# gnosisguild/pvw-rs

Measured on AMD Instinct MI355X. Metric: parties/s for n-party encrypt (pvw::crypto::encrypt); achieved HBM GB/s vs peak, higher is better.
Workload: dtype u64

## Files before the change

### include/pvw_hip.h

```cpp
#ifndef PVW_HIP_H
#define PVW_HIP_H

#include <stddef.h>
#include <stdint.h>

#if defined(__GNUC__)
#define PVW_API __attribute__((visibility("default")))
#else
#define PVW_API
#endif

#ifdef __cplusplus
extern "C" {
#endif

typedef struct pvw_ctx pvw_ctx;

enum {
  PVW_OK = 0,
  PVW_ERR_INVALID_PARAMETERS = 1,
  PVW_ERR_SAMPLING = 2,
  PVW_ERR_ENCRYPTION = 3,
  PVW_ERR_DECRYPTION = 4,
  PVW_ERR_KEY_GENERATION = 5,
// ... 209 lines not shown
PVW_API int32_t pvw_ntt_inverse(pvw_ctx* ctx, uint64_t* polys, size_t count);
PVW_API int32_t pvw_small_to_poly(pvw_ctx* ctx, const int64_t* coeffs, size_t count, uint64_t* polys,
                          uint32_t repr);

PVW_API int32_t pvw_sample_cbd(pvw_ctx* ctx, const uint8_t seed[32], uint32_t domain, uint32_t index0,
                       size_t count, float variance, int64_t* out);
PVW_API int32_t pvw_sample_uniform(pvw_ctx* ctx, const uint8_t seed[32], uint32_t domain,
                           uint32_t index0, size_t count, uint64_t bound, int64_t* out);
PVW_API int32_t pvw_sample_gaussian(pvw_ctx* ctx, const uint8_t seed[32], uint32_t index0, size_t count,
                            uint64_t bound, int64_t* out );

PVW_API int32_t pvw_ctx_set_profiling(pvw_ctx* ctx, int32_t on);
PVW_API int32_t pvw_ctx_kernel_time(pvw_ctx* ctx, const char* name, double* total_ms, uint64_t* launches);
PVW_API int32_t pvw_ctx_reset_profiling(pvw_ctx* ctx);
PVW_API int32_t pvw_host_alloc(size_t bytes, void** out);
PVW_API int32_t pvw_host_free(void* p);

PVW_API int32_t pvw_ctx_resident_bytes(const pvw_ctx* ctx, uint64_t* crs_bytes, uint64_t* pk_bytes);
PVW_API int32_t pvw_ctx_derived_bytes(const pvw_ctx* ctx, uint64_t* packed_bytes, uint64_t* mfma_tiled_bytes);

enum { PVW_PREPARE_PACKED = 1, PVW_PREPARE_MFMA = 2, PVW_PREPARE_SUM = 4 };
PVW_API int32_t pvw_prepare(pvw_ctx* ctx, uint32_t flags, void* stream, uint64_t* bytes_out);
PVW_API int32_t pvw_ctx_packed_active(const pvw_ctx* ctx, uint32_t* width_out);
PVW_API int32_t pvw_ctx_synchronize(pvw_ctx* ctx);

PVW_API int32_t pvw_wire_poly_bytes(const pvw_ctx* ctx, size_t* out);
PVW_API int32_t pvw_wire_header(const pvw_ctx* ctx, uint32_t kind, uint32_t repr, uint32_t lo, uint32_t hi, uint32_t lo2,
                                uint32_t hi2, uint8_t* out, size_t cap, size_t* len);
PVW_API int32_t pvw_wire_header_check(const pvw_ctx* ctx, const uint8_t* data, size_t len, uint32_t* kind, uint32_t* repr,
                                      uint32_t* ranges, size_t* header_len);
PVW_API int32_t pvw_wire_pack(pvw_ctx* ctx, const uint64_t* polys, size_t count, uint8_t* out);
PVW_API int32_t pvw_wire_pack_device(pvw_ctx* ctx, const uint64_t* d_polys, size_t count, uint8_t* d_out, void* stream);
PVW_API int32_t pvw_wire_unpack(pvw_ctx* ctx, const uint8_t* data, size_t count, uint64_t* polys);
PVW_API int32_t pvw_wire_unpack_device(pvw_ctx* ctx, const uint8_t* d_in, size_t count, uint64_t* d_polys, uint64_t* d_bad,
                                       void* stream);
PVW_API int32_t pvw_wire_pack_host(const pvw_ctx* ctx, const uint64_t* polys, size_t count, uint8_t* out);
PVW_API int32_t pvw_wire_unpack_host(const pvw_ctx* ctx, const uint8_t* data, size_t count, uint64_t* polys, uint64_t* bad_out);
PVW_API int32_t pvw_load_pk_wire(pvw_ctx* ctx, uint32_t party_lo, uint32_t party_hi, const uint8_t* body, uint32_t repr);
PVW_API int32_t pvw_get_pk_wire(pvw_ctx* ctx, uint32_t party_lo, uint32_t party_hi, uint8_t* body_out, uint32_t repr);
PVW_API int32_t pvw_load_crs_wire(pvw_ctx* ctx, const uint8_t* body, uint32_t repr);
PVW_API int32_t pvw_get_crs_wire(pvw_ctx* ctx, uint8_t* body_out, uint32_t repr);

#ifdef __cplusplus
}
#endif
#endif
// ... 1 lines not shown
```

### pvw_rs_amd/_ffi.py

```python
from __future__ import annotations

import ctypes as C
import os

HERE = os.path.dirname(os.path.abspath(__file__))
LIB_PATH = os.path.join(HERE, "libpvw_hip.so")

PVW_OK = 0
ERROR_NAMES = {
    1: "InvalidParameters", 2: "SamplingError", 3: "EncryptionError", 4: "DecryptionError",
    5: "KeyGenerationError", 6: "CrsError", 7: "SerializationError", 8: "DeserializationError",
    9: "EncodingError", 10: "DecodingError", 11: "ValidationError", 12: "ContextError",
    13: "PolynomialError", 14: "MatrixError", 15: "DimensionMismatch", 16: "IndexOutOfBounds",
    17: "InsufficientData", 18: "InvalidFormat", 19: "InternalError",
}
REPR_POWER, REPR_NTT = 0, 1
RND_SEED, RND_EXPLICIT = 0, 1
DOM_R, DOM_E1, DOM_E2, DOM_SK, DOM_EKEY, DOM_CRS, DOM_GAUSS, DOM_PK, DOM_CALL = range(9)
PREPARE_PACKED, PREPARE_MFMA, PREPARE_SUM = 1, 2, 4
WIRE_PARAMS, WIRE_CRS, WIRE_PK, WIRE_CT, WIRE_SK = 1, 2, 3, 4, 5


class pvw_params_t(C.Structure):
    _fields_ = [
# ... 86 lines not shown
    "pvw_selftest_decode_fixed": [_P, _P, C.c_size_t, _P],
    "pvw_selftest_mfma_i8": [_P, _P, _P, _P],
    "pvw_selftest_secret_residue": [_P, C.POINTER(C.c_uint64), C.POINTER(C.c_uint64)],
    "pvw_selftest_siphash": [_P, C.c_size_t, C.c_uint64, C.c_uint64, C.c_int32, C.c_int32, C.POINTER(C.c_uint64)],
    "pvw_selftest_decode_tables": [_P, C.POINTER(C.c_uint32)],
    "pvw_selftest_decode_shortcuts": [_P, _P, C.c_size_t, _P, _P],
    "pvw_build_is_tuning": [],
    "pvw_crs_seed_from_tag": [C.c_char_p, _P],
    "pvw_ntt_forward": [_P, _P, C.c_size_t],
    "pvw_ntt_inverse": [_P, _P, C.c_size_t],
    "pvw_small_to_poly": [_P, _P, C.c_size_t, _P, C.c_uint32],
    "pvw_sample_cbd": [_P, _P, C.c_uint32, C.c_uint32, C.c_size_t, C.c_float, _P],
    "pvw_sample_uniform": [_P, _P, C.c_uint32, C.c_uint32, C.c_size_t, C.c_uint64, _P],
    "pvw_sample_gaussian": [_P, _P, C.c_uint32, C.c_size_t, C.c_uint64, _P],
    "pvw_ctx_set_profiling": [_P, C.c_int32],
    "pvw_ctx_kernel_time": [_P, C.c_char_p, C.POINTER(C.c_double), C.POINTER(C.c_uint64)],
    "pvw_ctx_reset_profiling": [_P],
    "pvw_host_alloc": [C.c_size_t, C.POINTER(_P)],
    "pvw_host_free": [_P],
    "pvw_ctx_resident_bytes": [_P, C.POINTER(C.c_uint64), C.POINTER(C.c_uint64)],
    "pvw_ctx_derived_bytes": [_P, C.POINTER(C.c_uint64), C.POINTER(C.c_uint64)],
    "pvw_prepare": [_P, C.c_uint32, _P, C.POINTER(C.c_uint64)],
    "pvw_ctx_packed_active": [_P, C.POINTER(C.c_uint32)],
    "pvw_ctx_synchronize": [_P],
    "pvw_wire_poly_bytes": [_P, C.POINTER(C.c_size_t)],
    "pvw_wire_header": [_P, C.c_uint32, C.c_uint32, C.c_uint32, C.c_uint32, C.c_uint32, C.c_uint32, _P, C.c_size_t,
                        C.POINTER(C.c_size_t)],
    "pvw_wire_header_check": [_P, _P, C.c_size_t, C.POINTER(C.c_uint32), C.POINTER(C.c_uint32), _P, C.POINTER(C.c_size_t)],
    "pvw_wire_pack": [_P, _P, C.c_size_t, _P],
    "pvw_wire_pack_device": [_P, _P, C.c_size_t, _P, _P],
    "pvw_wire_unpack": [_P, _P, C.c_size_t, _P],
    "pvw_wire_unpack_device": [_P, _P, C.c_size_t, _P, _P, _P],
    "pvw_wire_pack_host": [_P, _P, C.c_size_t, _P],
    "pvw_wire_unpack_host": [_P, _P, C.c_size_t, _P, C.POINTER(C.c_uint64)],
    "pvw_load_pk_wire": [_P, C.c_uint32, C.c_uint32, _P, C.c_uint32],
    "pvw_get_pk_wire": [_P, C.c_uint32, C.c_uint32, _P, C.c_uint32],
    "pvw_load_crs_wire": [_P, _P, C.c_uint32],
    "pvw_get_crs_wire": [_P, _P, C.c_uint32],
}

_TUNING_SIGNATURES = {
    "pvw_selftest_read_bandwidth": [_P, C.c_uint32, _P, _P],
    "pvw_tuning_read_stamps": [_P, _P, _P, C.c_uint32],
    "pvw_tuning_read_probe": [_P, C.c_uint32, C.c_uint32, C.c_uint32, C.c_uint32, _P, _P],
}

# ... 45 lines not shown
```

### pvw_rs_amd/api.py

```python
from __future__ import annotations

import ctypes as C
import struct
from typing import List, Optional, Sequence, Tuple

import numpy as np

from . import _ffi
from ._ffi import REPR_NTT, REPR_POWER


class PvwError(Exception):

    def __init__(self, code: int, message: str):
        self.code = code
        self.variant = _ffi.ERROR_NAMES.get(code, f"Unknown({code})")
        super().__init__(f"{self.variant}: {message}")


def _check(rc: int, lib=None) -> None:
    if rc != _ffi.PVW_OK:
        raise PvwError(rc, _ffi.last_error(lib))


# ... 239 lines not shown

    def reset_profiling(self) -> None:
        self._call("pvw_ctx_reset_profiling")

    def kernel_time(self, name: str) -> Tuple[float, int]:
        ms, cnt = C.c_double(), C.c_uint64()
        self._call("pvw_ctx_kernel_time", name.encode(), C.byref(ms), C.byref(cnt))
        return ms.value, cnt.value

    def resident_bytes(self) -> Tuple[int, int]:
        a, b = C.c_uint64(), C.c_uint64()
        self._call("pvw_ctx_resident_bytes", C.byref(a), C.byref(b))
        return a.value, b.value

    def prepare(self, flags: int = _ffi.PREPARE_PACKED | _ffi.PREPARE_MFMA, stream=None) -> int:
        taken = C.c_uint64(0)
        self._call("pvw_prepare", int(flags), C.c_void_p(stream) if stream else None, C.byref(taken))
        return int(taken.value)

    def packed_active(self) -> int:
        w = C.c_uint32(0)
        self._call("pvw_ctx_packed_active", C.byref(w))
        return int(w.value)

    def derived_bytes(self) -> Tuple[int, int]:
        a, b = C.c_uint64(0), C.c_uint64(0)
        self._call("pvw_ctx_derived_bytes", C.byref(a), C.byref(b))
        return int(a.value), int(b.value)

    def synchronize(self) -> None:
        self._call("pvw_ctx_synchronize")

    def wire_poly_bytes(self) -> int:
        out = C.c_size_t()
        self._call("pvw_wire_poly_bytes", C.byref(out))
        return int(out.value)

    def to_bytes(self) -> bytes:
        return bytes(_wire_header(self, _ffi.WIRE_PARAMS))

    @staticmethod
    def from_bytes(data, device: int = -1) -> "PvwParameters":
        raw = bytes(data[:_WIRE_FIXED]) if len(data) >= _WIRE_FIXED else b""
        if len(raw) < _WIRE_FIXED or raw[:4] != _WIRE_MAGIC:
            raise PvwError(18, "wire: truncated header or bad magic")
        version, kind = struct.unpack_from("<HH", raw, 4)
# ... 898 lines not shown
```

### pvw_rs_amd/csrc/pvw_capi.hip

```cpp
#include <hip/hip_runtime.h>

#include <atomic>
#include <cmath>
#include <cstdio>
#include <cstring>
#include <functional>
#include <map>
#include <mutex>
#include <string>
#include <thread>
#include <vector>

#include "../../include/pvw_hip.h"
#include "pvw_arith.h"
#include "pvw_bignum.h"
#include "pvw_chacha.h"
#include "pvw_decode.h"
#include "pvw_kernels.h"
#if PVW_TUNING
#include "../../include/pvw_hip_tuning.h"
#endif

using namespace pvw;

// ... 135 lines not shown
  std::vector<u64> tw, itw, linv, ghat, gpow;
  bool roots_locked = false;
  std::vector<u64> dec_words;
  DecodeTables dec_host{};
  DecodeTables dec_dev{};
  void* d_dec = nullptr;

  std::atomic<bool> dev_ready{false};
  void* d_tables = nullptr;
  DevTables dt{};
  u64* dA = nullptr;
  u64* dB = nullptr;
  u64* xmA = nullptr;
  u64* xmB = nullptr;
  bool xm_valid = false;
  u64* pkA = nullptr;
  u64* pkB = nullptr;
  u32* pk_flag = nullptr;
  u32 pk_width = 0;
  bool pkA_valid = false, pkB_valid = false;
  bool pk_wide = false;
  u32 pk_nomem_calls = 0;
  bool crs_loaded = false;
  u32 num_keys = 0;
  hipStream_t stream = nullptr;

  std::mutex mu, init_mu;
  std::vector<Workspace*> pool;
  std::map<void*, Workspace*> async_ws;

  bool profiling = false;
  std::vector<ProfRec> prof;
  std::map<std::string, std::pair<double, uint64_t>> prof_acc;

  u32 rowsA() const { return c1_hi - c1_lo; }
  u32 rowsB() const { return party_hi - party_lo; }
  u32 R() const { return 128 / l; }
  size_t poly() const { return (size_t)L * l; }
  size_t tiled_words(u32 rows) const { return (size_t)((rows + R() - 1) / R()) * L * k * 128; }
};

struct ProfScope {
  pvw_ctx* c;
  hipStream_t s;
  ProfRec rec;
  bool on;
// ... 460 lines not shown
  pvw_ctx* c = new pvw_ctx();
  c->n = p->n; c->k = p->k; c->l = p->l; c->L = p->num_moduli;
  c->moduli.assign(p->moduli, p->moduli + p->num_moduli);
  c->variance = p->secret_variance;
  c->b1 = p->error_bound_1; c->b2 = p->error_bound_2;
  c->device = p->device;
  c->party_lo = p->party_lo; c->party_hi = p->party_hi;
  c->c1_lo = p->c1_lo; c->c1_hi = p->c1_hi;
  if (c->party_lo == 0 && c->party_hi == 0) c->party_hi = c->n;
  if (c->c1_lo == 0 && c->c1_hi == 0) c->c1_hi = c->k;
  if (c->party_lo > c->party_hi || c->party_hi > c->n || c->c1_lo > c->c1_hi || c->c1_hi > c->k) {
    delete c;
    return fail(PVW_ERR_INVALID_PARAMETERS, "party / c1 shard out of range");
  }
  compute_q_delta(c->moduli.data(), c->L, c->l, c->Q, c->delta, c->delta_pow);
  c->halfQ = c->Q.shr(1);
  for (u32 i = 0; i < c->L; ++i) {
    c->mods.push_back(make_mod(c->moduli[i]));
    c->psi.push_back(min_primitive_root(c->mods[i], 2 * c->l));
    BigInt qi = c->Q / BigInt(c->moduli[i]);
    c->crt_qi.push_back(qi);
    c->crt_inv.push_back(powmod(qi.mod_small(c->moduli[i]), c->moduli[i] - 2, c->mods[i]));
  }
  build_tables(c);
  build_decode_tables(c);
  {
    u32 maxbits = 0;
    for (u64 q : c->moduli) {
      u32 bits = 0;
      for (; q; q >>= 1) ++bits;
      if (bits > maxbits) maxbits = bits;
    }
    c->pk_width = packed_width(maxbits, c->k, c->l);
  }
  *out = c;
  return PVW_OK;
}

int32_t pvw_ctx_destroy(pvw_ctx* c) {
  if (!c) return PVW_OK;
  if (c->dev_ready) {
    hipSetDevice(c->device);
    hipDeviceSynchronize();
    for (auto& r : c->prof) { hipEventDestroy(r.a); hipEventDestroy(r.b); }
    for (Workspace* w : c->pool) ws_free(w);
    for (auto& kv : c->async_ws) ws_free(kv.second);
// ... 285 lines not shown
  PVW_TRY(device_ws(c, stream, &s, &w));
  size_t taken = 0;
  if (flags & PVW_PREPARE_SUM) PVW_TRY(sum_prepare(c, w, s));
  if (flags & PVW_PREPARE_PACKED) (void)ensure_packed(c, s, true, &taken);
  if (flags & PVW_PREPARE_MFMA) {
    const bool had_a = c->xmA != nullptr, had_b = c->xmB != nullptr;
    PVW_TRY(ws_gemm_buffers(c, w));
    PVW_TRY(ensure_xm(c, s));
    if (!had_a && c->xmA) taken += xm_words(c->rowsA(), c->k, c->L, c->l) * 8;
    if (!had_b && c->xmB) taken += xm_words(c->rowsB(), c->k, c->L, c->l) * 8;
  }
  PVW_HIP(hipStreamSynchronize(s));
  if (bytes_out) *bytes_out = taken;
  return PVW_OK;
}

static int32_t check_repr(uint32_t repr) {
  if (repr != PVW_REPR_POWER && repr != PVW_REPR_NTT) return fail(PVW_ERR_INVALID_FORMAT, "unknown representation");
  return PVW_OK;
}

static void matrix_changed(pvw_ctx* c, bool crs) {
  c->xm_valid = false;
  (crs ? c->pkA_valid : c->pkB_valid) = false;
  c->pk_wide = false;
}

int32_t pvw_load_crs(pvw_ctx* c, const uint64_t* a, uint32_t repr) {
  if (!c || !a) return fail(PVW_ERR_INVALID_PARAMETERS, "NULL argument");
  PVW_TRY(check_repr(repr));
  PVW_TRY(ensure_device(c));
  matrix_changed(c, true);
  PVW_TRY(ensure_matrix(c, &c->dA, c->rowsA()));
  PVW_TRY(load_rows_host(c, c->dA, c->c1_lo, c->c1_hi, 0, c->k, a, repr));
  c->crs_loaded = true;
  return PVW_OK;
}
int32_t pvw_load_crs_device(pvw_ctx* c, const uint64_t* d_a, uint32_t repr, void* stream) {
  if (!c || !d_a) return fail(PVW_ERR_INVALID_PARAMETERS, "NULL argument");
  PVW_TRY(check_repr(repr));
  PVW_TRY(ensure_device(c));
  matrix_changed(c, true);
  PVW_TRY(ensure_matrix(c, &c->dA, c->rowsA()));
  PVW_TRY(load_rows_device(c, c->dA, c->c1_lo, c->c1_hi, 0, c->k, d_a, repr, call_stream(c, stream)));
  c->crs_loaded = true;
  return PVW_OK;
}
int32_t pvw_crs_generate(pvw_ctx* c, const uint8_t seed[32]) {
  if (!c || !seed) return fail(PVW_ERR_INVALID_PARAMETERS, "NULL argument");
  PVW_TRY(ensure_device(c));
  matrix_changed(c, true);
  PVW_TRY(ensure_matrix(c, &c->dA, c->rowsA()));
  {
    ProfScope ps(c, "fill_uniform", c->stream);
    PVW_HIP(launch_fill_uniform_tiled(c->dA, make_key(seed), DOM_CRS, c->rowsA(), 0, c->c1_lo, c->k, c->L,
                                      c->l, c->dt, c->stream));
  }
  PVW_HIP(hipStreamSynchronize(c->stream));
  c->crs_loaded = true;
  return PVW_OK;
}
static u64 siphash(const uint8_t* m, size_t len, u64 k0, u64 k1, int c_rounds, int d_rounds) {
  u64 v0 = k0 ^ 0x736f6d6570736575ULL, v1 = k1 ^ 0x646f72616e646f6dULL, v2 = k0 ^ 0x6c7967656e657261ULL,
      v3 = k1 ^ 0x7465646279746573ULL;
  auto rotl = [](u64 x, int b) { return (x << b) | (x >> (64 - b)); };
  auto round = [&]() {
    v0 += v1; v1 = rotl(v1, 13); v1 ^= v0; v0 = rotl(v0, 32);
    v2 += v3; v3 = rotl(v3, 16); v3 ^= v2;
    v0 += v3; v3 = rotl(v3, 21); v3 ^= v0;
    v2 += v1; v1 = rotl(v1, 17); v1 ^= v2; v2 = rotl(v2, 32);
  };
  size_t i = 0;
  for (; i + 8 <= len; i += 8) {
    u64 w = 0;
    for (int b = 0; b < 8; ++b) w |= (u64)m[i + b] << (8 * b);
    v3 ^= w;
    for (int r = 0; r < c_rounds; ++r) round();
    v0 ^= w;
  }
  u64 w = (u64)(len & 0xff) << 56;
  for (int b = 0; i + b < len; ++b) w |= (u64)m[i + b] << (8 * b);
  v3 ^= w;
// ... 408 lines not shown
      pb.job[2].raw_out = w->esmall + (size_t)rA * l;
      es1 = pb.job[1].raw_out;
      es2 = pb.job[2].raw_out;
      pb.njobs = 3;
    }
  } else {
    pb.njobs = 3;
  }
  {
    ProfScope ps(c, "prologue", s);
    PVW_HIP(launch_prologue(pb, c->dt, L, l, s));
  }
  {
    ProfScope ps(c, "mac_rows", s);
    MacSection a(width ? c->pkA : c->dA, compact ? nullptr : d_c1, out_c1, rA), b(width ? c->pkB : c->dB, compact ? nullptr : d_c2, out_c2, rB);
    if (compact) {
      a.e_small = es1;
      b.e_small = es2;
      b.scalars = d_scalars + c->party_lo;
    }
    if (rs) {
      a.rnd_ctr = &rs->counter;
      a.rnd_adv = 1;
    }
    if (width) PVW_HIP(launch_mac_rows_packed(a, b, w->rhat, c->dt, k, L, l, width, s));
    else PVW_HIP(launch_mac_rows(a, b, w->rhat, c->dt, k, L, l, s));
  }
  if (out_repr == PVW_REPR_POWER) {
    ProfScope ps(c, "intt", s);
    PVW_HIP(launch_ntt(d_c1, rA, true, c->dt, L, l, s));
    PVW_HIP(launch_ntt(d_c2, rB, true, c->dt, L, l, s));
  }
  return PVW_OK;
}

int32_t pvw_encrypt_device(pvw_ctx* c, const uint64_t* d_scalars, size_t num_scalars, const pvw_randomness_t* rnd,
                           uint64_t* d_c1, uint64_t* d_c2, uint32_t out_repr, void* stream) {
  if (!c || !d_scalars || (!d_c1 && c->rowsA()) || (!d_c2 && c->rowsB())) return fail(PVW_ERR_INVALID_PARAMETERS, "NULL argument");
  PVW_TRY(encrypt_checks(c, num_scalars, rnd, out_repr));
  PVW_TRY(ensure_device(c));
  hipStream_t s;
  Workspace* w;
  PVW_TRY(device_ws(c, stream, &s, &w));
  return encrypt_enqueue(c, w, d_scalars, rnd, d_c1, d_c2, out_repr, s);
}

// ... 2052 lines not shown
```

### pvw_rs_amd/csrc/pvw_chacha.h

```cpp
#pragma once
#include "pvw_arith.h"

namespace pvw {

struct ChaChaKey {
  u32 w[8];
};

inline ChaChaKey make_key(const uint8_t seed[32]) {
  ChaChaKey k;
  for (int i = 0; i < 8; ++i)
    k.w[i] = (u32)seed[4 * i] | (u32)seed[4 * i + 1] << 8 | (u32)seed[4 * i + 2] << 16 |
             (u32)seed[4 * i + 3] << 24;
  return k;
}

PVW_HD u32 rotl32(u32 x, int n) { return (x << n) | (x >> (32 - n)); }

#define PVW_QR(a, b, c, d)                                                                   \
  a += b; d ^= a; d = rotl32(d, 16); c += d; b ^= c; b = rotl32(b, 12);                       \
  a += b; d ^= a; d = rotl32(d, 8);  c += d; b ^= c; b = rotl32(b, 7);

struct ChaChaRng {
  u32 key[8];
// ... 23 lines not shown
      PVW_QR(x2, x7, x8, x13) PVW_QR(x3, x4, x9, x14)
    }
    buf[0] = x0 + 0x61707865; buf[1] = x1 + 0x3320646e; buf[2] = x2 + 0x79622d32; buf[3] = x3 + 0x6b206574;
    buf[4] = x4 + key[0]; buf[5] = x5 + key[1]; buf[6] = x6 + key[2]; buf[7] = x7 + key[3];
    buf[8] = x8 + key[4]; buf[9] = x9 + key[5]; buf[10] = x10 + key[6]; buf[11] = x11 + key[7];
    buf[12] = x12 + (u32)counter; buf[13] = x13 + (u32)(counter >> 32); buf[14] = x14 + s0; buf[15] = x15 + s1;
    ++counter;
    pos = 0;
  }
  PVW_HD u32 next_u32() {
    if (pos == 16) refill();
    u32 v = 0;
#pragma unroll
    for (int i = 0; i < 16; ++i) v = (i == pos) ? buf[i] : v;
    ++pos;
    return v;
  }
  PVW_HD u64 next_u64() {
    u64 lo = next_u32();
    u64 hi = next_u32();
    return lo | (hi << 32);
  }
};

template <class Emit>
PVW_HD void sample_cbd_poly(ChaChaRng& g, u32 l, bool half, u32 v, Emit emit) {
  if (half && g.pos == 16) {
    for (u32 s0 = 0; s0 < l; s0 += 8) {
      g.refill();
#pragma unroll
      for (int i = 0; i < 8; ++i)
        if (s0 + i < l) emit(s0 + i, (i64)(g.buf[2 * i] & 1) - (i64)(g.buf[2 * i + 1] & 1));
      const u32 used = (l - s0) < 8 ? 2 * (l - s0) : 16;
      g.pos = (int)used;
    }
    return;
  }
  if (half) {
    for (u32 s = 0; s < l; ++s) {
      i64 b1 = g.next_u32() & 1;
      i64 b2 = g.next_u32() & 1;
      emit(s, b1 - b2);
    }
    return;
  }
  u32 nbits = 4 * v;
// ... 90 lines not shown
```

### pvw_rs_amd/csrc/pvw_kernels.h

```cpp
#pragma once
#include <hip/hip_runtime.h>

#include "pvw_arith.h"
#include "pvw_chacha.h"
#include "pvw_decode.h"

#ifndef PVW_TUNING
#define PVW_TUNING 0
#endif
#if PVW_TUNING
#include <cstdlib>
#define PVW_ENV_INT(name, dflt) ([]() -> long { const char* e_ = getenv(name); return e_ ? atol(e_) : (long)(dflt); }())
#else
#define PVW_ENV_INT(name, dflt) ((long)(dflt))
#endif

namespace pvw {

enum { DOM_R = 0, DOM_E1 = 1, DOM_E2 = 2, DOM_SK = 3, DOM_EKEY = 4, DOM_CRS = 5, DOM_GAUSS = 6, DOM_PK = 7, DOM_CALL = 8 };

struct RndState {
  u32 seed[8];
  u64 counter;
  u64 base;
// ... 34 lines not shown
struct SampleJob {
  u32 kind;
  u32 domain;
  u32 index0;
  u32 count;
  u32 out_poly0;
  u32 cbd_half;
  u32 cbd_v;
  u64 bound;
};

struct MacSection {
  const u64* M = nullptr;
  const u64* addend = nullptr;
  u64* out = nullptr;
  u32 nrows = 0;
  u32 row_blocks = 0;
  MacSection() = default;
  MacSection(const u64* M_, const u64* addend_, u64* out_, u32 nrows_) : M(M_), addend(addend_), out(out_), nrows(nrows_) {}
  const i64* e_small = nullptr;
  const u64* scalars = nullptr;
  u64* rnd_ctr = nullptr;
  u64 rnd_adv = 0;
};
hipError_t launch_prep(const i64* coeffs, const u64* scalars, u64* out, size_t stride_poly,
                       size_t stride_limb, u32 count, bool do_ntt, const DevTables& t, u32 L,
                       u32 ell, hipStream_t s, u32 group = 0, size_t stride_group = 0);
hipError_t launch_transpose_polys(const u64* src, u64* dst, u32 k, u32 words, hipStream_t s);
hipError_t launch_ntt(u64* polys, size_t count, bool inverse, const DevTables& t, u32 L, u32 ell,
                      hipStream_t s);
hipError_t launch_tile(const u64* src, u64* M, u32 rows, u32 row0_tiled, u32 k, u32 L, u32 ell,
                       bool ntt_first, const DevTables& t, hipStream_t s);
hipError_t launch_untile(const u64* M, u64* dst, u32 rows, u32 row0_tiled, u32 k, u32 L, u32 ell,
                         bool intt_after, const DevTables& t, hipStream_t s);
hipError_t launch_fill_uniform_tiled(u64* M, const ChaChaKey& key, u32 domain, u32 rows,
                                     u32 row0_tiled, u32 grow0, u32 k, u32 L, u32 ell,
                                     const DevTables& t, hipStream_t s);
struct PrologueJob {
  SampleJob sj;
  const i64* explicit_coeffs;
  const u64* scalars;
  u64* out;
  size_t stride_poly, stride_limb;
  u32 key_idx;
  u32 rep_key;
  u32 rep_index0;
  size_t rep_out, rep_scalars, rep_coeffs;
// ... 137 lines not shown
```

### pvw_rs_amd/csrc/pvw_mac.hip

```cpp
#include <hip/hip_runtime.h>

#include "pvw_arith.h"
#include "pvw_chacha.h"
#include "pvw_dev.h"
#include "pvw_kernels.h"

namespace pvw {

#if PVW_TUNING
#define PVW_STAMP_MAX 65536
__device__ u64 g_stamp_buf[2 * PVW_STAMP_MAX];
__device__ u32 g_stamp_hw[PVW_STAMP_MAX];
#endif
template <bool STAMP>
__device__ __forceinline__ void stamp_begin(u32 item) {
#if PVW_TUNING
  if constexpr (STAMP) {
    if (threadIdx.x == 0 && item < PVW_STAMP_MAX) {
      g_stamp_buf[2 * item] = __builtin_amdgcn_s_memrealtime();
      g_stamp_hw[item] = (__builtin_amdgcn_s_getreg(20 | (0 << 6) | (3 << 11)) << 28) | ((blockIdx.x & 7u) << 24) |
                         (__builtin_amdgcn_s_getreg(4 | (0 << 6) | (31 << 11)) & 0x00ffffffu);
    }
  }
#endif
// ... 148 lines not shown
    if (out_row < it.nrows) {
      v2u64 s = mac_partials_sum(lds, lane, m);
      if (it.has_addend()) {
        s.x = addmod(s.x, add_pf.x, m.q);
        s.y = addmod(s.y, add_pf.y, m.q);
      }
      reinterpret_cast<v2u64*>(it.out)[out_o] = s;
    }
  }
}
template <int ELL, bool STAMP>
__device__ __forceinline__ void mac_finish(MacFrame<ELL>& f, const DevTables& t, v2u64* lds, typename SmallAddend<ELL>::Lds& adl) {
  const Mod m = t.mods[f.limb];
  if constexpr (ELL <= 16) {
    if (f.wave == 0 && f.it.e_small) f.add_pf = mac_small_make<ELL>(f.it, t, m, f.small, f.lane, f.rho, f.sp, adl.w);
  }
  v2u64 part;
  part.x = acc_reduce(f.a0, m);
  part.y = acc_reduce(f.a1, m);
  mac_epilogue(lds, part, m, f.it, f.wave, f.lane, f.out_row, f.out_o, f.add_pf);
  stamp_end<STAMP>(f.item);
}

template <int ELL, int U, bool ILV = false, bool STAMP = false>
__global__ __launch_bounds__(256) void mac_rows_kernel(MacSection sa, MacSection sb, const u64* __restrict__ rhat, DevTables t, u32 k, u32 L) {
  constexpr int NW = 4;
  constexpr int HALF = ELL / 2;
  constexpr int JC = ELL <= 16 ? 64 : (ELL == 32 ? 32 : 16);
  __shared__ v2u64 lds[NW * JC * HALF];
  __shared__ typename SmallAddend<ELL>::Lds adl;
  static_assert(JC * HALF >= 64, "the wave partials reuse the r-hat slabs");
  MacFrame<ELL> f;
  mac_frame<ELL, STAMP>(f, sa, sb, rhat, k, L, lds, JC * HALF);
  const u32 wave = f.wave, lane = f.lane, sp = f.sp;
  const u32 kq = ILV ? k / NW : (k + NW - 1) / NW;
  const u32 j0 = ILV ? 0 : (wave * kq < k ? wave * kq : k);
  const u32 j1 = ILV ? kq : ((j0 + kq) < k ? (j0 + kq) : k);
  auto gmap = [&](u32 tt) -> u32 { return ILV ? (tt / U) * NW * U + wave * U + tt % U : tt; };

  const v2u64* Mp = reinterpret_cast<const v2u64*>(f.it.M + ((size_t)f.it.rb * L + f.limb) * (size_t)k * 128) + lane;
  const v2u64* rp = f.rp;
  v2u64* lw = f.lw;
  Acc &a0 = f.a0, &a1 = f.a1;

  for (u32 jc = j0; jc < j1; jc += JC) {
    const u32 cnt = (j1 - jc) < (u32)JC ? (j1 - jc) : (u32)JC;
    auto ld = [&](u32 tile) -> v2u64 { return __builtin_nontemporal_load(Mp + (size_t)gmap(jc + tile) * 64); };
    __builtin_amdgcn_wave_barrier();
    v2u64 x[U];
    const bool full = cnt >= U;
    if (full) {
#pragma unroll
      for (int u = 0; u < U; ++u) x[u] = ld(u);
    }
    if (jc == j0) mac_addend_request(f);
    constexpr int RN = JC * HALF / 64;
// ... 46 lines not shown
}

#ifndef PVW_PACKED_WPC
#define PVW_PACKED_WPC 2
#endif
template <int N>
__device__ __forceinline__ u64 pk_word(const v2u64 (&a)[N], int idx) { return (idx & 1) ? a[idx >> 1].y : a[idx >> 1].x; }
template <int W, int N>
__device__ __forceinline__ u64 pk_get(const v2u64 (&a)[N], int bit) {
  const int idx = bit >> 6, sh = bit & 63;
  u64 v = pk_word(a, idx) >> sh;
  if (sh + W > 64) v |= pk_word(a, idx + 1) << (64 - sh);
  return v & ((1ull << W) - 1);
}
template <int ELL, bool STAMP = false>
__global__ __launch_bounds__(256, PVW_PACKED_WPC) void mac_rows_packed61_kernel(MacSection sa, MacSection sb, const u64* __restrict__ rhat,
                                                                               DevTables t, u32 k, u32 L) {
  constexpr int HALF = ELL / 2, JC = 64, NW = 4, W = 61;
  static_assert(ELL <= 16, "one period of 64 j per r-hat slab");
  __shared__ v2u64 lds[NW * JC * HALF];
  __shared__ typename SmallAddend<ELL>::Lds adl;
  MacFrame<ELL> f;
  mac_frame<ELL, STAMP>(f, sa, sb, rhat, k, L, lds, JC * HALF);
  const u32 wave = f.wave, lane = f.lane, sp = f.sp;
  const u32 kq = k / NW, periods = kq / 64;
  const u32 chunks = k / 64 * W;
  const v2u64* Pp = reinterpret_cast<const v2u64*>(f.it.M) + (((size_t)f.it.rb * L + f.limb) * chunks + (size_t)wave * periods * W) * 64 + lane;
  const v2u64* rp = f.rp + (size_t)wave * kq * HALF;
  v2u64* lw = f.lw;
  Acc &a0 = f.a0, &a1 = f.a1;
  auto ldc = [&](u32 c) -> v2u64 { return __builtin_nontemporal_load(Pp + (size_t)c * 64); };
  v2u64 xa[16], xb[16];
#pragma unroll
  for (int u = 0; u < 16; ++u) xa[u] = ldc(u);
  mac_addend_request(f);
  for (u32 pd = 0; pd < periods; ++pd) {
    const u32 cb = pd * W;
    __builtin_amdgcn_wave_barrier();
    constexpr int RN = JC * HALF / 64;
    v2u64 rv[RN];
#pragma unroll
    for (int x = 0; x < RN; ++x) rv[x] = rp[(size_t)pd * 64 * HALF + lane + 64 * x];
#pragma unroll
    for (int x = 0; x < RN; ++x) lw[lane + 64 * x] = rv[x];
    __builtin_amdgcn_fence(__ATOMIC_RELEASE, "wavefront");
    __builtin_amdgcn_wave_barrier();
// ... 12 lines not shown
        const v2u64 r = lw[(16 * g + jj) * HALF + sp];
        acc_mac_dev(a0, xv, r.x);
        acc_mac_dev(a1, yv, r.y);
      }
      if (g < 3) nxt[0] = cur[15];
    };
    group(0, xa, xb);
    group(1, xb, xa);
    group(2, xa, xb);
    group(3, xb, xa);
  }
  mac_finish<ELL, STAMP>(f, t, lds, adl);
}

template <int ELL, int W, bool STAMP = false>
__global__ __launch_bounds__(256, PVW_PACKED_WPC) void mac_rows_packedw_kernel(MacSection sa, MacSection sb, const u64* __restrict__ rhat,
                                                                              DevTables t, u32 k, u32 L) {
  constexpr int HALF = ELL / 2, JC = 64, NW = 4, CG = W / 4;
  static_assert(ELL <= 16 && W % 4 == 0 && W < 64, "whole chunks per group");
  __shared__ v2u64 lds[NW * JC * HALF];
  __shared__ typename SmallAddend<ELL>::Lds adl;
  MacFrame<ELL> f;
  mac_frame<ELL, STAMP>(f, sa, sb, rhat, k, L, lds, JC * HALF);
  const u32 wave = f.wave, lane = f.lane, sp = f.sp;
  const u32 kq = k / NW, gw = kq / 16;
  const u32 chunks = k / 16 * CG;
  const v2u64* Pp = reinterpret_cast<const v2u64*>(f.it.M) + (((size_t)f.it.rb * L + f.limb) * chunks + (size_t)wave * gw * CG) * 64 + lane;
  const v2u64* rp = f.rp + (size_t)wave * kq * HALF;
  v2u64* lw = f.lw;
  Acc &a0 = f.a0, &a1 = f.a1;
  auto ldc = [&](u32 c) -> v2u64 { return __builtin_nontemporal_load(Pp + (size_t)c * 64); };
  v2u64 xa[CG], xb[CG];
#pragma unroll
  for (int u = 0; u < CG; ++u) xa[u] = ldc(u);
  mac_addend_request(f);
  auto group = [&](const u32 g, v2u64 (&cur)[CG], v2u64 (&nxt)[CG]) {
    constexpr int RN = JC * HALF / 64;
    const bool slab = (g & 3) == 0;
    v2u64 rv[RN];
    if (slab) {
      const u32 cnt = (gw - g) < 4 ? (gw - g) * 16 : 64;
      __builtin_amdgcn_wave_barrier();
#pragma unroll
      for (int x = 0; x < RN; ++x) {
        const u32 idx = lane + 64 * x;
        rv[x] = rp[(size_t)g * 16 * HALF + (idx < cnt * HALF ? idx : 0)];
// ... 345 lines not shown
```

### rust/pvw-hip-sys/src/lib.rs

```rust
#![allow(non_camel_case_types)]

use std::os::raw::{c_char, c_void};

#[repr(C)]
pub struct PvwCtx {
    _private: [u8; 0],
}

#[repr(C)]
pub struct PvwSk {
    _private: [u8; 0],
}

#[repr(C)]
#[derive(Debug, Clone, Copy)]
pub struct PvwParamsT {
    pub n: u32,
    pub k: u32,
    pub l: u32,
    pub num_moduli: u32,
    pub moduli: *const u64,
    pub secret_variance: f32,
    pub error_bound_1: u64,
    pub error_bound_2: u64,
// ... 127 lines not shown
    pub fn pvw_selftest_decode_fixed(ctx: *const PvwCtx, noisy: *const u64, count: usize, out_u64: *mut u64) -> i32;
    pub fn pvw_selftest_mfma_i8(ctx: *mut PvwCtx, a: *const i8, b: *const i8, out: *mut i32) -> i32;
    pub fn pvw_selftest_secret_residue(ctx: *mut PvwCtx, nonzero_words: *mut u64, scanned_words: *mut u64) -> i32;
    pub fn pvw_selftest_siphash(msg: *const u8, len: usize, k0: u64, k1: u64, c_rounds: i32, d_rounds: i32, out: *mut u64) -> i32;
    pub fn pvw_selftest_decode_tables(ctx: *const PvwCtx, info_out: *mut u32) -> i32;
    pub fn pvw_selftest_decode_shortcuts(ctx: *const PvwCtx, noisy: *const u64, count: usize, out_u64: *mut u64, short_path: *mut u8) -> i32;
    pub fn pvw_selftest_rnd_free_residue(nonzero_words: *mut u64) -> i32;
    pub fn pvw_build_is_tuning() -> i32;
    pub fn pvw_ntt_forward(ctx: *mut PvwCtx, polys: *mut u64, count: usize) -> i32;
    pub fn pvw_ntt_inverse(ctx: *mut PvwCtx, polys: *mut u64, count: usize) -> i32;
    pub fn pvw_small_to_poly(ctx: *mut PvwCtx, coeffs: *const i64, count: usize, polys: *mut u64, repr: u32) -> i32;
    pub fn pvw_sample_cbd(ctx: *mut PvwCtx, seed: *const u8, domain: u32, index0: u32, count: usize, variance: f32, out: *mut i64) -> i32;
    pub fn pvw_sample_uniform(ctx: *mut PvwCtx, seed: *const u8, domain: u32, index0: u32, count: usize, bound: u64, out: *mut i64) -> i32;
    pub fn pvw_sample_gaussian(ctx: *mut PvwCtx, seed: *const u8, index0: u32, count: usize, bound: u64, out: *mut i64) -> i32;
    pub fn pvw_ctx_set_profiling(ctx: *mut PvwCtx, on: i32) -> i32;
    pub fn pvw_ctx_kernel_time(ctx: *mut PvwCtx, name: *const c_char, total_ms: *mut f64, launches: *mut u64) -> i32;
    pub fn pvw_ctx_reset_profiling(ctx: *mut PvwCtx) -> i32;
    pub fn pvw_host_alloc(bytes: usize, out: *mut *mut c_void) -> i32;
    pub fn pvw_host_free(p: *mut c_void) -> i32;
    pub fn pvw_ctx_resident_bytes(ctx: *const PvwCtx, crs_bytes: *mut u64, pk_bytes: *mut u64) -> i32;
    pub fn pvw_ctx_derived_bytes(ctx: *const PvwCtx, packed_bytes: *mut u64, mfma_tiled_bytes: *mut u64) -> i32;
    pub fn pvw_prepare(ctx: *mut PvwCtx, flags: u32, stream: *mut c_void, bytes_out: *mut u64) -> i32;
    pub fn pvw_ctx_packed_active(ctx: *const PvwCtx, width_out: *mut u32) -> i32;
    pub fn pvw_ctx_synchronize(ctx: *mut PvwCtx) -> i32;
    pub fn pvw_wire_poly_bytes(ctx: *const PvwCtx, out: *mut usize) -> i32;
    pub fn pvw_wire_header(ctx: *const PvwCtx, kind: u32, repr: u32, lo: u32, hi: u32, lo2: u32, hi2: u32, out: *mut u8, cap: usize, len: *mut usize) -> i32;
    pub fn pvw_wire_header_check(ctx: *const PvwCtx, data: *const u8, len: usize, kind: *mut u32, repr: *mut u32, ranges: *mut u32, header_len: *mut usize) -> i32;
    pub fn pvw_wire_pack(ctx: *mut PvwCtx, polys: *const u64, count: usize, out: *mut u8) -> i32;
    pub fn pvw_wire_pack_device(ctx: *mut PvwCtx, d_polys: *const u64, count: usize, d_out: *mut u8, stream: *mut c_void) -> i32;
    pub fn pvw_wire_unpack(ctx: *mut PvwCtx, data: *const u8, count: usize, polys: *mut u64) -> i32;
    pub fn pvw_wire_unpack_device(ctx: *mut PvwCtx, d_in: *const u8, count: usize, d_polys: *mut u64, d_bad: *mut u64, stream: *mut c_void) -> i32;
    pub fn pvw_wire_pack_host(ctx: *const PvwCtx, polys: *const u64, count: usize, out: *mut u8) -> i32;
    pub fn pvw_wire_unpack_host(ctx: *const PvwCtx, data: *const u8, count: usize, polys: *mut u64, bad_out: *mut u64) -> i32;
    pub fn pvw_load_pk_wire(ctx: *mut PvwCtx, party_lo: u32, party_hi: u32, body: *const u8, repr: u32) -> i32;
    pub fn pvw_get_pk_wire(ctx: *mut PvwCtx, party_lo: u32, party_hi: u32, body_out: *mut u8, repr: u32) -> i32;
    pub fn pvw_load_crs_wire(ctx: *mut PvwCtx, body: *const u8, repr: u32) -> i32;
    pub fn pvw_get_crs_wire(ctx: *mut PvwCtx, body_out: *mut u8, repr: u32) -> i32;
}
```

Before: 21.52 million.

## Regenerate seeded CRS matrix on the fly inside MAC kernel instead of loading it

When the CRS was generated from a seed and the moduli pass a rejection-rate gate, the A-matrix MAC path regenerates each CRS limb element in-kernel with a quad-lane ChaCha8 block using DPP permutes. It falls back to a full sequential replay only when a lane's sample is rejected. This replaces HBM reads of the large CRS matrix with ALU work, trading a memory-bound stream for compute. It adds env switches, a query API, and invalidation when the CRS changes.

Measured after the change: 20.40 million. 0.948x the previous value.

```diff
diff --git a/include/pvw_hip.h b/include/pvw_hip.h
--- a/include/pvw_hip.h
+++ b/include/pvw_hip.h
@@ -255,6 +255,7 @@
 enum { PVW_PREPARE_PACKED = 1, PVW_PREPARE_MFMA = 2, PVW_PREPARE_SUM = 4 };
 PVW_API int32_t pvw_prepare(pvw_ctx* ctx, uint32_t flags, void* stream, uint64_t* bytes_out);
 PVW_API int32_t pvw_ctx_packed_active(const pvw_ctx* ctx, uint32_t* width_out);
+PVW_API int32_t pvw_ctx_crs_seeded(const pvw_ctx* ctx, uint32_t* seeded_out);
 PVW_API int32_t pvw_ctx_synchronize(pvw_ctx* ctx);
 
 PVW_API int32_t pvw_wire_poly_bytes(const pvw_ctx* ctx, size_t* out);
diff --git a/pvw_rs_amd/_ffi.py b/pvw_rs_amd/_ffi.py
--- a/pvw_rs_amd/_ffi.py
+++ b/pvw_rs_amd/_ffi.py
@@ -132,6 +132,7 @@
     "pvw_ctx_derived_bytes": [_P, C.POINTER(C.c_uint64), C.POINTER(C.c_uint64)],
     "pvw_prepare": [_P, C.c_uint32, _P, C.POINTER(C.c_uint64)],
     "pvw_ctx_packed_active": [_P, C.POINTER(C.c_uint32)],
+    "pvw_ctx_crs_seeded": [_P, C.POINTER(C.c_uint32)],
     "pvw_ctx_synchronize": [_P],
     "pvw_wire_poly_bytes": [_P, C.POINTER(C.c_size_t)],
     "pvw_wire_header": [_P, C.c_uint32, C.c_uint32, C.c_uint32, C.c_uint32, C.c_uint32, C.c_uint32, _P, C.c_size_t,
diff --git a/pvw_rs_amd/api.py b/pvw_rs_amd/api.py
--- a/pvw_rs_amd/api.py
+++ b/pvw_rs_amd/api.py
@@ -285,6 +285,11 @@
         w = C.c_uint32(0)
         self._call("pvw_ctx_packed_active", C.byref(w))
         return int(w.value)
+
+    def crs_seeded(self) -> bool:
+        w = C.c_uint32(0)
+        self._call("pvw_ctx_crs_seeded", C.byref(w))
+        return bool(w.value)
 
     def derived_bytes(self) -> Tuple[int, int]:
         a, b = C.c_uint64(0), C.c_uint64(0)
diff --git a/pvw_rs_amd/csrc/pvw_capi.hip b/pvw_rs_amd/csrc/pvw_capi.hip
--- a/pvw_rs_amd/csrc/pvw_capi.hip
+++ b/pvw_rs_amd/csrc/pvw_capi.hip
@@ -181,6 +181,9 @@
   bool pk_wide = false;
   u32 pk_nomem_calls = 0;
   bool crs_loaded = false;
+  bool crs_seeded = false;
+  ChaChaKey crs_key{};
+  bool crs_moduli_ok = false;
   u32 num_keys = 0;
   hipStream_t stream = nullptr;
 
@@ -687,6 +690,8 @@
     c->crt_qi.push_back(qi);
     c->crt_inv.push_back(powmod(qi.mod_small(c->moduli[i]), c->moduli[i] - 2, c->mods[i]));
   }
+  c->crs_moduli_ok = true;
+  for (u32 i = 0; i < c->L; ++i) c->crs_moduli_ok = c->crs_moduli_ok && crs_seed_modulus_ok(c->moduli[i]);
   build_tables(c);
   build_decode_tables(c);
   {
@@ -1018,6 +1023,7 @@
 
 static void matrix_changed(pvw_ctx* c, bool crs) {
   c->xm_valid = false;
+  if (crs) c->crs_seeded = false;
   (crs ? c->pkA_valid : c->pkB_valid) = false;
   c->pk_wide = false;
 }
@@ -1054,6 +1060,18 @@
   }
   PVW_HIP(hipStreamSynchronize(c->stream));
   c->crs_loaded = true;
+  c->crs_key = make_key(seed);
+  c->crs_seeded = true;
+  return PVW_OK;
+}
+static bool crs_seed_active(const pvw_ctx* c) {
+  if (!c->crs_seeded || (c->l != 8 && c->l != 16) || c->rowsA() == 0) return false;
+  if (PVW_ENV_INT("PVW_MAC_CRS_SEED", 1) == 0) return false;
+  return c->crs_moduli_ok || PVW_ENV_INT("PVW_MAC_CRS_GATE", 1) == 0;
+}
+int32_t pvw_ctx_crs_seeded(const pvw_ctx* c, uint32_t* seeded_out) {
+  if (!c || !seeded_out) return fail(PVW_ERR_INVALID_PARAMETERS, "NULL argument");
+  *seeded_out = crs_seed_active(c) ? 1 : 0;
   return PVW_OK;
 }
 static u64 siphash(const uint8_t* m, size_t len, u64 k0, u64 k1, int c_rounds, int d_rounds) {
@@ -1508,6 +1526,11 @@
     if (rs) {
       a.rnd_ctr = &rs->counter;
       a.rnd_adv = 1;
+    }
+    if (crs_seed_active(c)) {
+      a.seeded = true;
+      a.crs_key = c->crs_key;
+      a.crs_row0 = c->c1_lo;
     }
     if (width) PVW_HIP(launch_mac_rows_packed(a, b, w->rhat, c->dt, k, L, l, width, s));
     else PVW_HIP(launch_mac_rows(a, b, w->rhat, c->dt, k, L, l, s));
diff --git a/pvw_rs_amd/csrc/pvw_chacha.h b/pvw_rs_amd/csrc/pvw_chacha.h
--- a/pvw_rs_amd/csrc/pvw_chacha.h
+++ b/pvw_rs_amd/csrc/pvw_chacha.h
@@ -69,6 +69,85 @@
     return lo | (hi << 32);
   }
 };
+
+#if defined(__HIPCC__)
+#define PVW_QUAD_FN PVW_D
+constexpr int QUAD_LANES = 1;
+PVW_D u32 quad_lane(int) { return threadIdx.x & 3; }
+#define PVW_QUAD_PERM(s0, s1, s2, s3) ((s0) | (s1) << 2 | (s2) << 4 | (s3) << 6)
+template <int CTRL>
+PVW_D u32 quad_perm(u32 v) { return (u32)__builtin_amdgcn_update_dpp((int)v, (int)v, CTRL, 0xf, 0xf, false); }
+template <int D>
+PVW_D void quad_rot(u32 (&v)[1]) {
+  static_assert(D >= 1 && D <= 3, "rotation within the quad");
+  v[0] = quad_perm<PVW_QUAD_PERM(D & 3, (D + 1) & 3, (D + 2) & 3, (D + 3) & 3)>(v[0]);
+}
+template <int X>
+PVW_D void quad_xor(u32 (&v)[1]) {
+  static_assert(X == 1 || X == 2, "partner within the quad");
+  v[0] = quad_perm<PVW_QUAD_PERM(X, 1 ^ X, 2 ^ X, 3 ^ X)>(v[0]);
+}
+#else
+#define PVW_QUAD_FN inline
+constexpr int QUAD_LANES = 4;
+inline u32 quad_lane(int i) { return (u32)i; }
+template <int D>
+inline void quad_rot(u32 (&v)[4]) {
+  const u32 t[4] = {v[D & 3], v[(D + 1) & 3], v[(D + 2) & 3], v[(D + 3) & 3]};
+  for (int c = 0; c < 4; ++c) v[c] = t[c];
+}
+template <int X>
+inline void quad_xor(u32 (&v)[4]) {
+  const u32 t[4] = {v[X], v[1 ^ X], v[2 ^ X], v[3 ^ X]};
+  for (int c = 0; c < 4; ++c) v[c] = t[c];
+}
+#endif
+template <int X>
+PVW_QUAD_FN void quad_swap(u32 (&lo)[QUAD_LANES], u32 (&hi)[QUAD_LANES]) {
+  u32 t[QUAD_LANES];
+#pragma unroll
+  for (int i = 0; i < QUAD_LANES; ++i) t[i] = (quad_lane(i) & X) ? lo[i] : hi[i];
+  quad_xor<X>(t);
+#pragma unroll
+  for (int i = 0; i < QUAD_LANES; ++i) {
+    if (quad_lane(i) & X) lo[i] = t[i];
+    else hi[i] = t[i];
+  }
+}
+PVW_QUAD_FN u32 quad_pick(u32 c, u32 v0, u32 v1, u32 v2, u32 v3) { return c == 0 ? v0 : (c == 1 ? v1 : (c == 2 ? v2 : v3)); }
+PVW_QUAD_FN void chacha8_block_quad(const ChaChaKey& key, u32 domain, u32 stream, u64 block, u32 (&out)[QUAD_LANES][4]) {
+  u32 a0[QUAD_LANES], b0[QUAD_LANES], c0[QUAD_LANES], d0[QUAD_LANES];
+  u32 a[QUAD_LANES], b[QUAD_LANES], c[QUAD_LANES], d[QUAD_LANES];
+#pragma unroll
+  for (int i = 0; i < QUAD_LANES; ++i) {
+    const u32 col = quad_lane(i);
+    a[i] = a0[i] = quad_pick(col, 0x61707865, 0x3320646e, 0x79622d32, 0x6b206574);
+    b[i] = b0[i] = quad_pick(col, key.w[0], key.w[1], key.w[2], key.w[3]);
+    c[i] = c0[i] = quad_pick(col, key.w[4], key.w[5], key.w[6], key.w[7]);
+    d[i] = d0[i] = quad_pick(col, (u32)block, (u32)(block >> 32), stream, domain);
+  }
+#pragma unroll
+  for (int r = 0; r < 4; ++r) {
+#pragma unroll
+    for (int i = 0; i < QUAD_LANES; ++i) { PVW_QR(a[i], b[i], c[i], d[i]) }
+    quad_rot<1>(b);
+    quad_rot<2>(c);
+    quad_rot<3>(d);
+#pragma unroll
+    for (int i = 0; i < QUAD_LANES; ++i) { PVW_QR(a[i], b[i], c[i], d[i]) }
+    quad_rot<3>(b);
+    quad_rot<2>(c);
+    quad_rot<1>(d);
+  }
+#pragma unroll
+  for (int i = 0; i < QUAD_LANES; ++i) { a[i] += a0[i]; b[i] += b0[i]; c[i] += c0[i]; d[i] += d0[i]; }
+  quad_swap<1>(a, b);
+  quad_swap<1>(c, d);
+  quad_swap<2>(a, c);
+  quad_swap<2>(b, d);
+#pragma unroll
+  for (int i = 0; i < QUAD_LANES; ++i) { out[i][0] = a[i]; out[i][1] = b[i]; out[i][2] = c[i]; out[i][3] = d[i]; }
+}
 
 template <class Emit>
 PVW_HD void sample_cbd_poly(ChaChaRng& g, u32 l, bool half, u32 v, Emit emit) {
diff --git a/pvw_rs_amd/csrc/pvw_kernels.h b/pvw_rs_amd/csrc/pvw_kernels.h
--- a/pvw_rs_amd/csrc/pvw_kernels.h
+++ b/pvw_rs_amd/csrc/pvw_kernels.h
@@ -80,7 +80,14 @@
   const u64* scalars = nullptr;
   u64* rnd_ctr = nullptr;
   u64 rnd_adv = 0;
-};
+  ChaChaKey crs_key{};
+  u32 crs_row0 = 0;
+  bool seeded = false;
+};
+inline bool crs_seed_modulus_ok(u64 q) {
+  const u32 w = 64 - (u32)__builtin_clzll(q);
+  return w >= 32 && ((w == 64 ? 0 : (u64)1 << w) - q) <= ((u64)1 << (w - 32));
+}
 hipError_t launch_prep(const i64* coeffs, const u64* scalars, u64* out, size_t stride_poly,
                        size_t stride_limb, u32 count, bool do_ntt, const DevTables& t, u32 L,
                        u32 ell, hipStream_t s, u32 group = 0, size_t stride_group = 0);
diff --git a/pvw_rs_amd/csrc/pvw_mac.hip b/pvw_rs_amd/csrc/pvw_mac.hip
--- a/pvw_rs_amd/csrc/pvw_mac.hip
+++ b/pvw_rs_amd/csrc/pvw_mac.hip
@@ -194,6 +194,75 @@
   stamp_end<STAMP>(f.item);
 }
 
+template <int ELL>
+__device__ __forceinline__ void mac_rows_seeded(MacFrame<ELL>& f, const MacSection& sa, const DevTables& t, u32 k, u32 L) {
+  static_assert(ELL == 8 || ELL == 16, "a polynomial limb is one or two whole blocks");
+  constexpr int HALF = ELL / 2, JC = 64, NW = 4, RN = JC * HALF / 64;
+  const u32 lane = f.lane, sp = f.sp;
+  const u32 kq = (k + NW - 1) / NW;
+  const u32 j0 = f.wave * kq < k ? f.wave * kq : k;
+  const u32 j1 = (j0 + kq) < k ? (j0 + kq) : k;
+  const u64 q = t.mods[f.limb].q;
+  const u32 sh = (u32)__clzll((long long)q);
+  const u32 blk = sp / 4;
+  const u32 pshift = f.rho * HALF;
+  const u32 s_row = (sa.crs_row0 + f.out_row) * k * L + f.limb;
+  const v2u64* rp = f.rp;
+  v2u64* lw = f.lw;
+  mac_addend_request(f);
+  auto draw = [&](u32 stream, u64& x, u64& y) -> bool {
+    u32 w[QUAD_LANES][4];
+    chacha8_block_quad(sa.crs_key, DOM_CRS, stream, blk, w);
+    x = ((u64)w[0][0] | (u64)w[0][1] << 32) >> sh;
+    y = ((u64)w[0][2] | (u64)w[0][3] << 32) >> sh;
+    return x >= q || y >= q;
+  };
+  auto replay = [&](u64 rejected, u32 stream, u64& x, u64& y) {
+    if (((rejected >> pshift) & ((1ull << HALF) - 1)) == 0) return;
+    ChaChaRng g;
+    g.init(sa.crs_key, DOM_CRS, stream);
+    for (u32 s = 0; s < (u32)ELL; ++s) {
+      u64 v;
+      do { v = g.next_u64() >> sh; } while (v >= q);
+      if (s == 2 * sp) x = v;
+      if (s == 2 * sp + 1) y = v;
+    }
+  };
+  for (u32 jc = j0; jc < j1; jc += JC) {
+    const u32 cnt = (j1 - jc) < (u32)JC ? (j1 - jc) : (u32)JC;
+    __builtin_amdgcn_wave_barrier();
+    v2u64 rv[RN];
+#pragma unroll
+    for (int x = 0; x < RN; ++x) {
+      const u32 idx = lane + 64 * x;
+      rv[x] = rp[(size_t)jc * HALF + (idx < cnt * HALF ? idx : 0)];
+    }
+#pragma unroll
+    for (int x = 0; x < RN; ++x) lw[lane + 64 * x] = rv[x];
+    __builtin_amdgcn_fence(__ATOMIC_RELEASE, "wavefront");
+    __builtin_amdgcn_wave_barrier();
+    for (u32 jj = 0; jj < cnt; jj += 2) {
+      const bool two = jj + 1 < cnt;
+      const u32 s0 = s_row + (jc + jj) * L, s1 = s0 + L;
+      u64 x0, y0, x1, y1;
+      const bool b0 = draw(s0, x0, y0);
+      const bool b1 = draw(s1, x1, y1);
+      const u64 rej0 = __ballot(b0), rej1 = __ballot(b1);
+      if (rej0 | rej1) {
+        replay(rej0, s0, x0, y0);
+        replay(rej1, s1, x1, y1);
+      }
+      if (!two) x1 = y1 = 0;
+      const v2u64 r0 = lw[jj * HALF + sp];
+      const v2u64 r1 = lw[(jj + (two ? 1 : 0)) * HALF + sp];
+      acc_mac_dev(f.a0, x0, r0.x);
+      acc_mac_dev(f.a1, y0, r0.y);
+      acc_mac_dev(f.a0, x1, r1.x);
+      acc_mac_dev(f.a1, y1, r1.y);
+    }
+  }
+}
+
 template <int ELL, int U, bool ILV = false, bool STAMP = false>
 __global__ __launch_bounds__(256) void mac_rows_kernel(MacSection sa, MacSection sb, const u64* __restrict__ rhat, DevTables t, u32 k, u32 L) {
   constexpr int NW = 4;
@@ -204,6 +273,13 @@
   static_assert(JC * HALF >= 64, "the wave partials reuse the r-hat slabs");
   MacFrame<ELL> f;
   mac_frame<ELL, STAMP>(f, sa, sb, rhat, k, L, lds, JC * HALF);
+  if constexpr (ELL <= 16) {
+    if (f.it.in_a && sa.seeded) {
+      mac_rows_seeded<ELL>(f, sa, t, k, L);
+      mac_finish<ELL, STAMP>(f, t, lds, adl);
+      return;
+    }
+  }
   const u32 wave = f.wave, lane = f.lane, sp = f.sp;
   const u32 kq = ILV ? k / NW : (k + NW - 1) / NW;
   const u32 j0 = ILV ? 0 : (wave * kq < k ? wave * kq : k);
@@ -296,6 +372,13 @@
   __shared__ typename SmallAddend<ELL>::Lds adl;
   MacFrame<ELL> f;
   mac_frame<ELL, STAMP>(f, sa, sb, rhat, k, L, lds, JC * HALF);
+  if constexpr (ELL <= 16) {
+    if (f.it.in_a && sa.seeded) {
+      mac_rows_seeded<ELL>(f, sa, t, k, L);
+      mac_finish<ELL, STAMP>(f, t, lds, adl);
+      return;
+    }
+  }
   const u32 wave = f.wave, lane = f.lane, sp = f.sp;
   const u32 kq = k / NW, periods = kq / 64;
   const u32 chunks = k / 64 * W;
@@ -354,6 +437,13 @@
   __shared__ typename SmallAddend<ELL>::Lds adl;
   MacFrame<ELL> f;
   mac_frame<ELL, STAMP>(f, sa, sb, rhat, k, L, lds, JC * HALF);
+  if constexpr (ELL <= 16) {
+    if (f.it.in_a && sa.seeded) {
+      mac_rows_seeded<ELL>(f, sa, t, k, L);
+      mac_finish<ELL, STAMP>(f, t, lds, adl);
+      return;
+    }
+  }
   const u32 wave = f.wave, lane = f.lane, sp = f.sp;
   const u32 kq = k / NW, gw = kq / 16;
   const u32 chunks = k / 16 * CG;
diff --git a/rust/pvw-hip-sys/src/lib.rs b/rust/pvw-hip-sys/src/lib.rs
--- a/rust/pvw-hip-sys/src/lib.rs
+++ b/rust/pvw-hip-sys/src/lib.rs
@@ -173,6 +173,7 @@
     pub fn pvw_ctx_derived_bytes(ctx: *const PvwCtx, packed_bytes: *mut u64, mfma_tiled_bytes: *mut u64) -> i32;
     pub fn pvw_prepare(ctx: *mut PvwCtx, flags: u32, stream: *mut c_void, bytes_out: *mut u64) -> i32;
     pub fn pvw_ctx_packed_active(ctx: *const PvwCtx, width_out: *mut u32) -> i32;
+    pub fn pvw_ctx_crs_seeded(ctx: *const PvwCtx, seeded_out: *mut u32) -> i32;
     pub fn pvw_ctx_synchronize(ctx: *mut PvwCtx) -> i32;
     pub fn pvw_wire_poly_bytes(ctx: *const PvwCtx, out: *mut usize) -> i32;
     pub fn pvw_wire_header(ctx: *const PvwCtx, kind: u32, repr: u32, lo: u32, hi: u32, lo2: u32, hi2: u32, out: *mut u8, cap: usize, len: *mut usize) -> i32;
```
